# elizabethfong/SparkSmithWaterman

Hardware: AMD Instinct MI355X
Metric: GCUPS (higher is better)
Workload: dtype int32

## Files before the change

### sparksmithwaterman_amd/csrc/swmi_ctx.cpp

```cpp
#include <cstdarg>
#include <cstdio>
#include <cstdlib>

#include "swmi_host.h"
#include "swmi_launch.h"

static thread_local std::string g_err;

int swmi_host::fail(int code, const char *fmt, ...) {
    char buf[512];
    va_list ap;
    va_start(ap, fmt);
    vsnprintf(buf, sizeof buf, fmt, ap);
    va_end(ap);
    g_err = buf;
    return code;
}

int swmi_io_fail(int code, const std::string &msg) { return fail(code, "%s", msg.c_str()); }

static const uint8_t *code_table();

extern "C" int swmi_abi_version(void) { return SWMI_ABI_VERSION; }

// ... 131 lines not shown
        if (value != -1 && value != 1) return fail(SWMI_ERR_INVALID, "affine must be -1 (when gap_open != 0) or 1 (always)");
        ctx->affine = (int)value;
    } else if (!strcmp(name, "align_mode")) {
        if (value != SWMI_ALIGN_LOCAL && value != SWMI_ALIGN_FIT && value != SWMI_ALIGN_GLOBAL)
            return fail(SWMI_ERR_INVALID, "align_mode must be 0 (local), 1 (fit) or 2 (global), got %lld", (long long)value);
        ctx->modes.align_mode = (int)value;
    } else if (!strcmp(name, "long_reads")) {
        if (value != 0 && value != 1) return fail(SWMI_ERR_INVALID, "long_reads must be 0 or 1, got %lld", (long long)value);
        ctx->modes.long_reads = (int)value;
    } else if (!strcmp(name, "band")) {
        if (value < 0 || value > (int64_t)SWMI_AFF_BAND_MAX)
            return fail(SWMI_ERR_INVALID, "band must be 0 (none) or a half-width of 1 .. %u columns, got %lld", SWMI_AFF_BAND_MAX, (long long)value);
        ctx->modes.band = (int)value;
    } else if (!strcmp(name, "extend")) {
        if (value != 0 && value != 1) return fail(SWMI_ERR_INVALID, "extend must be 0 or 1, got %lld", (long long)value);
        ctx->modes.extend = (int)value;
    } else if (!strcmp(name, "xdrop")) {
        if (value < 0 || value > 0x7FFFFFFFll)
            return fail(SWMI_ERR_INVALID, "xdrop must be 0 (off) or a threshold of 1 .. 2^31 - 1, got %lld", (long long)value);
        ctx->modes.xdrop = (int)value;
    } else if (!strcmp(name, "band_adapt")) {
        if (value != 0 && value != 1) return fail(SWMI_ERR_INVALID, "band_adapt must be 0 or 1, got %lld", (long long)value);
        ctx->modes.band_adapt = (int)value;
    } else if (!strcmp(name, "arena_words_per_pair")) {
        if (value < 1) return fail(SWMI_ERR_INVALID, "arena_words_per_pair out of range");
        ctx->arena_words_per_pair = (uint64_t)value;
    } else {
        return fail(SWMI_ERR_INVALID, "unknown option '%s'", name);
    }
    return SWMI_OK;
}

extern "C" int swmi_set_score_matrix(swmi_ctx *ctx, const uint8_t *alphabet, uint32_t n, const int32_t *scores) {
    if (!ctx) return fail(SWMI_ERR_INVALID, "null context");
    if (n == 0) {
        std::lock_guard<std::mutex> g(ctx->mat_mu);
        ctx->matrix.reset();
        return SWMI_OK;
    }
    if (n > SWMI_MAT_MAX_SYMBOLS) return fail(SWMI_ERR_INVALID, "a score matrix has at most %u symbols, got %u", SWMI_MAT_MAX_SYMBOLS, n);
    if (!alphabet || !scores) return fail(SWMI_ERR_INVALID, "alphabet or scores is null");
    const uint8_t *T = code_table();
    uint32_t cls[256];
    for (uint32_t c = 0; c < 256; c++) cls[c] = n;
    for (uint32_t i = 0; i < n; i++) {
        const uint8_t c = T[alphabet[i]];
// ... 143 lines not shown
```

### sparksmithwaterman_amd/csrc/swmi_device.h

```cpp
#pragma once
#include <stdint.h>

#if defined(__HIPCC__)
#define SWMI_HD __host__ __device__
#else
#define SWMI_HD
#endif

#define SWMI_SEQ_PAD_WORDS 24u
#define SWMI_RMAX          4
#ifndef SWMI_CK_BLOCKS
#define SWMI_CK_BLOCKS     2u
#endif
#define SWMI_CODE_PAD      0x1FFu

#define SWMI_LDS_BYTES (160u * 1024u)
#define SWMI_EMIT_SCRATCH_WORDS 128u
#define SWMI_TB_BLOCKS 16u
#define SWMI_TB_REFWIN_WORDS 96u
#define SWMI_RES_CELL_CAP 128u

#define SWMI_DIR_D 0u
#define SWMI_DIR_I 1u
#define SWMI_DIR_A 2u

#define SWMI_F_DEGENERATE   0x1u
#define SWMI_F_CELL_OVF     0x2u
#define SWMI_F_ARENA_OVF    0x4u
#define SWMI_F_DONE         0x8u
#define SWMI_F_STRIPS_SHIFT 8u
#define SWMI_F_STRIPS_MASK  0xFFFFFF00u

struct SeqDesc {
    uint32_t len;
    uint32_t boff;
    uint32_t acgt;
    uint32_t pad;
};

struct PairDesc {
    uint32_t ref_id;
    uint32_t read_id;
// ... 244 lines not shown
```

### sparksmithwaterman_amd/csrc/swmi_diag.cpp

```cpp
#include <chrono>
#include <cstdio>
#include <cstdlib>
#include <unistd.h>

#include "swmi_host.h"

int swmi_host::dump_traceback_diagnostics(swmi_batch *b, const TraceArgs &ta, size_t np, size_t n_tf) {
    if (!ta.dbg) return SWMI_OK;
    std::vector<unsigned long long> d(np * 4);
    HIP_TRY(hipMemcpy(d.data(), ta.dbg, np * 32, hipMemcpyDeviceToHost));
    if (n_tf) {
        double t0 = 0, t1 = 0, t2 = 0, t3 = 0, t4 = 0, t5 = 0; unsigned long long mx = 0;
        for (size_t k = 0; k < np; k++) {
            t0 += d[4*k]; t1 += d[4*k+1] & 0xFFFFFFFFull; t2 += d[4*k+1] >> 32; t3 += d[4*k+2] >> 16; t4 += d[4*k+3] >> 32; t5 += d[4*k+3] & 0xFFFFFFFFull;
            mx = std::max(mx, d[4*k]);
        }
        fprintf(stderr, "[swmi tfused dbg] ticks per sweeper wavefront: lifetime mean=%.0f max=%llu = prologue %.0f + sweep %.0f + first block task %.0f (%.2f block tasks per wavefront) + waiting for tasks %.0f + rest (more tasks, walk items) %.0f\n",
                t0 / np, mx, t2 / np, t1 / np, t3 / np, t5 / np, t4 / np, (t0 - t1 - t2 - t3 - t4) / np);
        {
            std::vector<size_t> idx(np);
            for (size_t k = 0; k < np; k++) idx[k] = k;
            std::sort(idx.begin(), idx.end(), [&](size_t x, size_t y) { return d[4 * x] < d[4 * y]; });
            auto at = [&](double q) { return d[4 * idx[std::min<size_t>(np - 1, (size_t)(q * np))]]; };
            fprintf(stderr, "[swmi tfused dbg]   lifetime p10=%llu p50=%llu p90=%llu p99=%llu max=%llu\n", at(0.10), at(0.50), at(0.90), at(0.99), d[4 * idx[np - 1]]);
            for (size_t t = 0; t < std::min<size_t>(np, 6); t++) {
                const size_t k = idx[np - 1 - t];
                fprintf(stderr, "[swmi tfused dbg]   slow wavefront (pair %zu): lifetime %llu, sweep %llu, first block task %llu, block tasks taken %llu, waiting %llu, alignments of its pair %llu\n",
                        k, d[4 * k], d[4 * k + 1] & 0xFFFFFFFFull, d[4 * k + 2] >> 16, d[4 * k + 3] & 0xFFFFFFFFull, d[4 * k + 3] >> 32,
                        (unsigned long long)((const PairOut *)((const uint8_t *)b->h_result.p + result_out_off()))[k].n_cells);
            }
        }
    }
    double a0 = 0, a1 = 0, a2 = 0, a3 = 0; unsigned long long mx = 0;
    double a4 = 0;
    for (size_t k = 0; k < np; k++) { a0 += d[4*k]; a1 += d[4*k+1] & 0xFFFFFFFFull; a2 += d[4*k+2] & 0xFFFF; a4 += d[4*k+2] >> 16; a3 += d[4*k+3] & 0xFFFFFFFFull; mx = std::max(mx, d[4*k]); }
    fprintf(stderr, "[swmi tb dbg] wave ticks mean=%.0f max=%llu; walk ticks mean=%.0f; staging ticks mean=%.0f; steps mean=%.1f; iterations mean=%.2f\n",
            a0 / np, mx, a1 / np, a4 / np, a2 / np, a3 / np);
    const PairOut *po_dbg = (const PairOut *)((const uint8_t *)b->h_result.p + result_out_off());
    double cs[4] = {0, 0, 0, 0}, cw[4] = {0, 0, 0, 0}; unsigned long long cm[4] = {0, 0, 0, 0}; size_t cn[4] = {0, 0, 0, 0};
    for (size_t k = 0; k < np; k++) {
        const size_t c = std::min<uint64_t>(po_dbg[k].n_cells, 4) - (po_dbg[k].n_cells ? 1 : 0);
        cs[c] += d[4 * k]; cw[c] += d[4 * k + 1] & 0xFFFFFFFFull; cm[c] = std::max(cm[c], d[4 * k]); cn[c]++;
    }
    {
        std::vector<size_t> idx(np);
        for (size_t k = 0; k < np; k++) idx[k] = k;
        const size_t top = std::min<size_t>(np, 6);
        std::partial_sort(idx.begin(), idx.begin() + top, idx.end(), [&](size_t x, size_t y) { return d[4 * x] > d[4 * y]; });
        for (size_t t = 0; t < top; t++)
            fprintf(stderr, "[swmi tb dbg]   slow pair %zu: ticks=%llu walk=%llu staging=%llu in %llu stagings, steps=%llu iterations=%llu alignments=%llu\n", idx[t],
                    d[4 * idx[t]], d[4 * idx[t] + 1] & 0xFFFFFFFFull, d[4 * idx[t] + 2] >> 16, d[4 * idx[t] + 3] >> 32, d[4 * idx[t] + 2] & 0xFFFF,
                    d[4 * idx[t] + 3] & 0xFFFFFFFFull, (unsigned long long)po_dbg[idx[t]].n_cells);
        for (size_t t = 0; t < top; t++)
            fprintf(stderr, "[swmi tb dbg]     ... of the staging time of pair %zu, %llu ticks waiting for helpers\n", idx[t], d[4 * idx[t] + 1] >> 32);
    }
    for (int c = 0; c < 4; c++)
        if (cn[c]) fprintf(stderr, "[swmi tb dbg]   %d%s alignment(s): %zu pairs, wave ticks mean=%.0f max=%llu, walk(slot 0) mean=%.0f\n",
                           c + 1, c == 3 ? "+" : "", cn[c], cs[c] / cn[c], cm[c], cw[c] / cn[c]);
    return SWMI_OK;
}

int swmi_host::dump_fill_diagnostics(swmi_batch *b, const FillArgs &fa, size_t np) {
    if (!fa.dbg) return SWMI_OK;
    std::vector<unsigned long long> d(np * 2);
    HIP_TRY(hipMemcpy(d.data(), fa.dbg, np * 16, hipMemcpyDeviceToHost));
#ifdef SWMI_STRIP_DIAG
    for (size_t k = 0; k < np && k < 8; k++)
        fprintf(stderr, "[swmi strip dbg] pair %zu: strip 0 lifetime %llu ticks, %llu waiting before publications; strip 1 lifetime %llu, "
                "%llu polls, %llu ticks in polls, %llu waiting for seam groups\n", k, d[2 * k] >> 32, d[2 * k] & 0xFFFFFFFFull,
                d[2 * k + 1] >> 40, (d[2 * k + 1] >> 32) & 0xFF, (d[2 * k + 1] >> 16) & 0xFFFF, d[2 * k + 1] & 0xFFFF);
#endif
    unsigned long long ev = 0, cyc = 0, evmax = 0, cmax = 0, cmin = ~0ull;
    for (size_t k = 0; k < np; k++) {
        ev += d[2 * k]; cyc += d[2 * k + 1];
        evmax = std::max(evmax, d[2 * k]); cmax = std::max(cmax, d[2 * k + 1]); cmin = std::min(cmin, d[2 * k + 1]);
    }
    fprintf(stderr, "[swmi fill dbg] pairs=%zu slow-path entries mean=%.1f max=%llu; wave ticks mean=%.0f min=%llu max=%llu\n",
// ... 32 lines not shown
```

### sparksmithwaterman_amd/csrc/swmi_host.h

```cpp
#pragma once
#include <hip/hip_runtime.h>

#include <algorithm>
#include <atomic>
#include <condition_variable>
#include <cstdint>
#include <cstring>
#include <memory>
#include <mutex>
#include <string>
#include <thread>
#include <type_traits>
#include <unordered_map>
#include <vector>

#include "../../include/swmi.h"
#include "swmi_device.h"
#include "swmi_io_internal.h"

namespace swmi_host __attribute__((visibility("hidden"))) {
int fail(int code, const char *fmt, ...);
int check_offsets(const uint64_t *off, uint32_t n, const char *what);
int upload_device(swmi_ctx *ctx, swmi_batch *b, hipStream_t st, const uint8_t *ref_src, const uint8_t *read_src);
int settle_raw(swmi_batch *b);
// ... 47 lines not shown
        return SWMI_OK;
    }
    void release() { if (p) (void)hipHostFree(p); p = nullptr; dp = nullptr; cap = 0; }
    PinnedBuf() = default;
    PinnedBuf(const PinnedBuf &) = delete;
    PinnedBuf &operator=(const PinnedBuf &) = delete;
    ~PinnedBuf() { release(); }
};

struct ScoreMatrix {
    uint64_t gen = 0;
    uint32_t n = 0;
    int32_t max_entry = 0;
    std::vector<uint32_t> image;
};

struct __attribute__((visibility("hidden"))) RunModes {
    int align_mode = SWMI_ALIGN_LOCAL;
    int long_reads = 0;
    int band = 0;
    int extend = 0;
    int xdrop = 0;
    int band_adapt = 0;
    uint32_t kernel_mode() const { return extend && align_mode == SWMI_ALIGN_GLOBAL ? 3u : (uint32_t)align_mode; }
    bool operator==(const RunModes &o) const { return memcmp(this, &o, sizeof(RunModes)) == 0; }
};
static_assert(std::has_unique_object_representations_v<RunModes>, "RunModes is compared bytewise: no padding, no floating point");
static inline int64_t swmi_adapt_low(uint64_t m, uint64_t n, int64_t gap_open, int64_t gap) {
    const int64_t ns = (int64_t)((m + SWMI_AFF_MAX_READ - 1) / SWMI_AFF_MAX_READ);
    return (2 * ns + 1) * gap_open + (ns * (int64_t)SWMI_AFF_MAX_READ + (int64_t)n) * gap;
}
static inline bool swmi_adapt_bound_ok(uint64_t m, uint64_t n, int64_t gap_open, int64_t gap) {
    return swmi_adapt_low(m, n, gap_open, gap) >= -((int64_t)1 << 30);
}
struct __attribute__((visibility("hidden"))) RunOptions {
    RunModes modes;
    std::shared_ptr<const ScoreMatrix> mat;
};

struct swmi_ctx {
    int device = 0;
    hipStream_t stream = nullptr;
    std::mutex mu;
    uint32_t cell_cap = 64;
    uint64_t max_workspace_bytes = 32ull << 30;
    int profiling = 0;
// ... 193 lines not shown
```

### sparksmithwaterman_amd/csrc/swmi_run.cpp

```cpp
#include <chrono>
#include <cstdio>
#include <cstdlib>
#include <functional>
#include <numeric>

#include "swmi_host.h"
#include "swmi_launch.h"
#include "swmi_plan.h"

static int keep_chunk_records(RunState &rs, const AlnRec *tab, uint64_t n_rec, const uint32_t *arena, uint64_t arena_cap, size_t lo) {
    swmi_batch *b = rs.b;
    if (rs.defer_copy && b->raw_chunks.empty()) {
        b->raw_ext = arena; b->rtab_ext = tab; b->raw_ext_records = n_rec; b->raw_ext_cap = arena_cap;
        b->raw_chunks.push_back(swmi_batch::RawChunk{0, 0, 0, (size_t)n_rec, lo, {}});
        return SWMI_OK;
    }
    uint64_t used = 0;
    for (uint64_t k = 0; k < n_rec; k++) {
        const uint64_t end = (((uint64_t)tab[k].off_hi << 32) | tab[k].off_lo) + rec_words(tab[k].n_ops, b->rec_strings);
        used = std::max(used, end);
    }
    if (used > arena_cap) return fail(SWMI_ERR_HIP, "record payloads overrun the arena");
    b->raw_chunks.push_back(swmi_batch::RawChunk{b->raw.size(), (size_t)used, b->rtab.size(), (size_t)n_rec, lo, {}});
    b->raw.insert(b->raw.end(), arena, arena + used);
// ... 100 lines not shown
    return SWMI_OK;
}

static int build_trace_args(RunState &rs, Launch &L) {
    swmi_ctx *ctx = rs.ctx;
    swmi_batch *b = rs.b;
    const ChunkPlan &plan = b->plan;
    const FillArgs &fa = rs.fa;
    int rc;
    TraceArgs &ta = rs.ta;
    ta.seqw = fa.seqw; ta.refs = fa.refs; ta.reads = fa.reads; ta.pairs = fa.pairs;
    ta.dir = fa.dir; ta.out = fa.out; ta.cells = fa.cells;
    ta.cells_off = fa.cells_off; ta.cells_cap = fa.cells_cap;
    ta.hdr = (ArenaHdr *)L.res;
    ta.arena = (uint32_t *)(L.res + L.a_off);
    ta.arena_cap_words = L.arena_cap;
    ta.rec_tab = (AlnRec *)(L.res + L.t_off);
    ta.rec_tab_cap = (uint32_t)std::min<uint64_t>(L.tab_cap, 0xFFFFFFFFu);
    ta.n_pairs = fa.n_pairs; ta.cell_cap = fa.cell_cap;
    ta.match = fa.match; ta.mismatch = fa.mismatch; ta.gap = fa.gap; ta.strict = fa.strict;
    ta.lds_words = (plan.max_path + 3) / 4 + 1;
    ta.seam = fa.seam;
    ta.mode = b->eff_mode;
    ta.pad2 = 0;
    ta.lds_read_words = (plan.max_read + 3) / 4 + 1;
    ta.out_host = nullptr;
    ta.ovf_host = (uint32_t *)ctx->h_err.dp + 4;
    ((volatile uint32_t *)ctx->h_err.p)[4] = 0u; ((volatile uint32_t *)ctx->h_err.p)[5] = 0u;
    ta.win_off = nullptr; ta.q_count = nullptr; ta.q_items = nullptr; ta.q_cap = 0; ta.pad4 = 0;
    const bool strings = ctx->device_strings != 0 && b->d_raw.p != nullptr;
    ta.raw = strings ? b->d_raw.as<uint8_t>() : nullptr;
    ta.raw_off = strings ? b->d_raw_off.as<uint64_t>() : nullptr;
    ta.raw_reads_at = b->n_refs + 1u;
    b->rec_strings = strings;
    if (L.zc) {
        if ((rc = b->h_result.reserve(L.a_off + L.arena_cap * 4))) return rc;
        uint8_t *hd = (uint8_t *)b->h_result.dp;
        *(volatile uint32_t *)b->h_result.p = 0u;
        ((volatile uint32_t *)b->h_result.p)[1] = 0u;
        ta.ovf_host = (uint32_t *)hd;
        ta.out_host = (PairOut *)(hd + result_out_off());
        ta.arena = (uint32_t *)(hd + L.a_off);
        ta.rec_tab = (AlnRec *)(hd + L.t_off);
    }
    ta.dbg = nullptr;
    if (dbg_fill_on()) {
        if ((rc = b->d_dbg2.reserve(L.np * 32))) return rc;
        HIP_TRY(hipMemsetAsync(b->d_dbg2.p, 0, L.np * 32, ctx->stream));
        ta.dbg = b->d_dbg2.as<unsigned long long>();
    }
    L.whole_only = L.zc && plan.n_tf + plan.n_res == L.np;
    if (L.whole_only) {
        const uint32_t slots = 1024;
        if (!ctx->d_hdr_ring.p || ctx->hdr_next >= slots) {
            if ((rc = ctx->d_hdr_ring.reserve((size_t)slots * 64))) return rc;
            HIP_TRY(hipMemsetAsync(ctx->d_hdr_ring.p, 0, (size_t)slots * 64, ctx->stream));
            ctx->hdr_next = 0;
        }
        ta.hdr = (ArenaHdr *)(ctx->d_hdr_ring.as<uint8_t>() + (size_t)ctx->hdr_next++ * 64);
    }
    return SWMI_OK;
}

static ResidentArgs resident_args(const swmi_batch *b) {
    const ChunkPlan &plan = b->plan;
    ResidentArgs xa;
    xa.res_items = plan.n_res ? b->d_res_items.as<uint32_t>() : nullptr;
    xa.n_res = (uint32_t)plan.n_res; xa.res_lds_words = plan.res_lds_words; xa.res_cell_cap = SWMI_RES_CELL_CAP; xa.res_ops_words = plan.res_ops_words;
    return xa;
}

// ... 699 lines not shown
```

### sparksmithwaterman_amd/csrc/swmi_traceback.hip

```cpp
#include <hip/hip_runtime.h>
#include <hip/hip_ext.h>
#include <stdint.h>
#include <stdlib.h>
#include "swmi_device.h"
#include "swmi_emit.h"
#include "swmi_launch.h"
#include "swmi_walk.h"

template <int R>
__device__ __forceinline__ void coop_helper(const TraceArgs &A, const PairDesc pd, const uint32_t lane, const uint32_t wave,
                                            const uint32_t nw, const uint32_t ts, const uint32_t n_waves_all,
                                            uint32_t *__restrict__ tiles, volatile uint32_t *__restrict__ shared) {
    const SeqDesc rd = A.refs[pd.ref_id];
    const SeqDesc qd = A.reads[pd.read_id];
    const uint32_t n = rd.len, m = qd.len;
    const uint32_t *__restrict__ refw = A.seqw + rd.boff;
    const uint32_t *__restrict__ readw = A.seqw + qd.boff;
    const StripGeom G = strip_geom<R>(m, n, 1u);
    const bool acgt = rd.acgt && qd.acgt && SWMI_SCORES_FIT(A);
    const uint32_t team = (wave - nw) % nw, q = 1u + (wave - nw) / nw;
    uint32_t last = 0;
    for (;;) {
        uint32_t seq;
        while ((seq = __hip_atomic_load(const_cast<uint32_t *>(&shared[7u + 4u * team]), __ATOMIC_RELAXED, __HIP_MEMORY_SCOPE_WORKGROUP)) == last)
            __builtin_amdgcn_s_sleep(SWMI_HELPER_SLEEP);
        if (seq == 0xFFFFFFFFu) break;
        last = seq;
        __builtin_amdgcn_fence(__ATOMIC_ACQUIRE, "workgroup");
        const uint32_t flags = shared[4u + 4u * team], wlo = shared[5u + 4u * team], nq = shared[6u + 4u * team];
        const uint32_t s = flags >> 2;
        const uint32_t win = (flags & 2u) ? q - 1u : q;
        if (q < ts && win < nq) {
            uint32_t *__restrict__ base = ((flags & 1u) ? tiles + n_waves_all * (SWMI_CK_BLOCKS * SWMI_RMAX * WAVE) : tiles) +
                                          team * ts * (SWMI_CK_BLOCKS * SWMI_RMAX * WAVE);
            (void)replay_any<R, false, false>(A, pd, n, m, acgt, refw, readw, G, s, wlo + win * SWMI_CK_BLOCKS, lane,
                                       base + win * SWMI_CK_BLOCKS * R * WAVE, 0, 0u, nullptr, 0u);
            __builtin_amdgcn_fence(__ATOMIC_RELEASE, "workgroup");
            if (lane == 0) atomicAdd(const_cast<uint32_t *>(&shared[20u + team]), 1u);
        }
    }
}

template <int TMODE>
__device__ __forceinline__ void traceback_entry(const TraceArgs &A, uint32_t *lds_all) {
    const uint32_t wave = threadIdx.x >> 6;
    const uint32_t pair = blockIdx.x * FILL_WAVES + wave;
    if (pair >= A.n_pairs) return;
    const uint32_t lane = threadIdx.x & 63u;
    const uint32_t slot = blockIdx.y;
    uint32_t *tb_lds = lds_all + wave * (A.lds_words + A.lds_read_words + SWMI_TB_REFWIN_WORDS +
                                         (TMODE == 0 ? SWMI_TB_BLOCKS : SWMI_CK_BLOCKS) * SWMI_RMAX * WAVE);
    uint32_t *tile = tb_lds + A.lds_words + A.lds_read_words + SWMI_TB_REFWIN_WORDS;
    const PairDesc pd = A.pairs[pair];
    const PairOut po = A.out[pd.out_id];
    if (A.out_host && slot == 0 && lane == 0) A.out_host[pd.out_id] = po;
    if (po.flags & (SWMI_F_DEGENERATE | SWMI_F_CELL_OVF)) return;
    if (po.n_cells <= slot) return;
// ... 119 lines not shown
    return (pre && wave == 0) ? wlo0 : 0xFFFFFFFFu;
}

extern "C" __global__ void __launch_bounds__(WAVE * SWMI_TB_WAVES) __attribute__((amdgpu_waves_per_eu(4, 4)))
sw_traceback_winmax_kernel(const TraceArgs A) {
    extern __shared__ uint32_t wm_lds[];
    const uint32_t pair = blockIdx.x;
    if (pair >= A.n_pairs) return;
    const uint32_t wave = threadIdx.x >> 6, lane = threadIdx.x & 63u;
    const PairDesc pd = A.pairs[pair];
    PairOut po = A.out[pd.out_id];
    if (finish_pair(A, pd, po) && wave == 0 && lane == 0) A.out[pd.out_id] = po;
    if (po.flags & (SWMI_F_DEGENERATE | SWMI_F_DONE)) {
        if (A.out_host && wave == 0 && lane == 0) A.out_host[pd.out_id] = po;
        return;
    }
    const uint32_t n_waves = blockDim.x >> 6;
    const uint32_t per_walker = A.lds_words + A.lds_read_words + SWMI_TB_REFWIN_WORDS;
    constexpr uint32_t WIN_WORDS = SWMI_CK_BLOCKS * SWMI_RMAX * WAVE;
    uint32_t *shared = wm_lds;
    uint32_t *tiles = wm_lds + 32;
    const uint32_t R = swmi_rows_per_lane(A.reads[pd.read_id].len);
    const uint32_t ccap = A.cells_cap ? A.cells_cap[pd.out_id] : A.cell_cap;
    const uint32_t tile_sets = A.pad2 ? 2u : 1u;
    uint32_t *tiles2 = A.pad2 ? tiles + n_waves * WIN_WORDS : nullptr;
    uint32_t *walker_lds0 = tiles + tile_sets * n_waves * WIN_WORDS;
    if (!swmi_common_pair(A, A.refs[pd.ref_id], A.reads[pd.read_id])) {
        if (wave == 0) {
            uint32_t c;
            if (R == 1)      c = detect_cells<1>(A, pd, po, lane, tiles);
            else if (R == 2) c = detect_cells<2>(A, pd, po, lane, tiles);
            else if (R == 3) c = detect_cells<3>(A, pd, po, lane, tiles);
            else             c = detect_cells<4>(A, pd, po, lane, tiles);
            if (lane == 0) {
                po.n_cells = c;
                if (c > ccap) po.flags |= SWMI_F_CELL_OVF;
                A.out[pd.out_id] = po;
                if (A.out_host) A.out_host[pd.out_id] = po;
                shared[0] = c;
            }
            asm volatile("s_waitcnt vmcnt(0)" ::: "memory");
        }
        __syncthreads();
        const uint32_t c = shared[0];
        uint32_t nwr = c < SWMI_TB_SLOTS ? c : SWMI_TB_SLOTS;
        if (nwr > n_waves) nwr = n_waves;
        if (c > ccap || wave >= nwr) return;
        po.n_cells = c;
        uint32_t *lds = walker_lds0 + wave * per_walker;
// ... 9 lines not shown
    else if (R == 2) pre_wlo = winmax_detect<2>(A, pd, po, lane, wave, n_waves, ccap, tiles, walker_lds0, per_walker, shared);
    else if (R == 3) pre_wlo = winmax_detect<3>(A, pd, po, lane, wave, n_waves, ccap, tiles, walker_lds0, per_walker, shared);
    else             pre_wlo = winmax_detect<4>(A, pd, po, lane, wave, n_waves, ccap, tiles, walker_lds0, per_walker, shared);
    const uint32_t cnt = shared[0];
    if (shared[3] != 1u) pre_wlo = 0xFFFFFFFFu;
    if (cnt > ccap || cnt == 0u) return;
    po.n_cells = cnt;
    uint32_t nw = cnt < SWMI_TB_SLOTS ? cnt : SWMI_TB_SLOTS;
    if (nw > n_waves) nw = n_waves;
    const uint32_t ts = n_waves / nw;
    if (ts == 1u) {
        if (wave >= nw) return;
        uint32_t *lds = walker_lds0 + wave * per_walker;
        uint32_t *tile = tiles + wave * WIN_WORDS;
        if (R == 1)      traceback_pair<1, 1, false, false>(A, pd, po, lane, wave, nw, lds, tile, nullptr, 1u, pre_wlo, true);
        else if (R == 2) traceback_pair<2, 1, false, false>(A, pd, po, lane, wave, nw, lds, tile, nullptr, 1u, pre_wlo, true);
        else if (R == 3) traceback_pair<3, 1, false, false>(A, pd, po, lane, wave, nw, lds, tile, nullptr, 1u, pre_wlo, true);
        else             traceback_pair<4, 1, false, false>(A, pd, po, lane, wave, nw, lds, tile, nullptr, 1u, pre_wlo, true);
        return;
    }
    if (wave < nw) {
        uint32_t *lds = walker_lds0 + wave * per_walker;
        uint32_t *tile = tiles + wave * ts * WIN_WORDS;
        uint32_t *tile2 = tiles2 ? tiles2 + wave * ts * WIN_WORDS : nullptr;
        if (R == 1)      traceback_pair<1, 1, true, false>(A, pd, po, lane, wave, nw, lds, tile, shared, ts, pre_wlo, true, nullptr, tile2);
        else if (R == 2) traceback_pair<2, 1, true, false>(A, pd, po, lane, wave, nw, lds, tile, shared, ts, pre_wlo, true, nullptr, tile2);
        else if (R == 3) traceback_pair<3, 1, true, false>(A, pd, po, lane, wave, nw, lds, tile, shared, ts, pre_wlo, true, nullptr, tile2);
        else             traceback_pair<4, 1, true, false>(A, pd, po, lane, wave, nw, lds, tile, shared, ts, pre_wlo, true, nullptr, tile2);
    } else {
        if (R == 1)      coop_helper<1>(A, pd, lane, wave, nw, ts, n_waves, tiles, shared);
        else if (R == 2) coop_helper<2>(A, pd, lane, wave, nw, ts, n_waves, tiles, shared);
        else if (R == 3) coop_helper<3>(A, pd, lane, wave, nw, ts, n_waves, tiles, shared);
        else             coop_helper<4>(A, pd, lane, wave, nw, ts, n_waves, tiles, shared);
    }
}

extern "C" __global__ void __launch_bounds__(WAVE * FILL_WAVES)
sw_traceback_kernel(const TraceArgs A) {
    extern __shared__ uint32_t tb_lds[];
    traceback_entry<0>(A, tb_lds);
}

extern "C" __global__ void __launch_bounds__(WAVE * FILL_WAVES)
sw_traceback_replay_kernel(const TraceArgs A) {
    extern __shared__ uint32_t tb_lds[];
    traceback_entry<1>(A, tb_lds);
}
// ... 307 lines not shown

extern "C" hipError_t swmi_launch_resident(const TraceArgs *a, const ResidentArgs *x, hipStream_t st) {
    if (x->n_res == 0) return hipSuccess;
    static const bool attr = [] { swmi_allow_big_lds(sw_resident_pairs_kernel); return true; }();
    (void)attr;
    hipLaunchKernelGGL(sw_resident_pairs_kernel, dim3((x->n_res + FILL_WAVES - 1) / FILL_WAVES), dim3(WAVE * FILL_WAVES),
                       (size_t)FILL_WAVES * x->res_lds_words * sizeof(uint32_t), st, *a, *x);
    return hipGetLastError();
}

extern "C" hipError_t swmi_launch_traceback(const TraceArgs *a, hipStream_t st, hipEvent_t ev_start, hipEvent_t ev_stop) {
    if (a->n_pairs == 0) return hipSuccess;
    const size_t tile = (size_t)(a->mode == 0 ? SWMI_TB_BLOCKS : SWMI_CK_BLOCKS) * SWMI_RMAX * WAVE;
    const size_t per_wave = (size_t)a->lds_words + a->lds_read_words + SWMI_TB_REFWIN_WORDS + tile;
    const dim3 block(WAVE * FILL_WAVES);
    if (a->mode == 1) {
        static int forced = getenv("SWMI_TB_WAVES") ? atoi(getenv("SWMI_TB_WAVES")) : 0;
        static int big = getenv("SWMI_TB_BIG") ? atoi(getenv("SWMI_TB_BIG")) : 10000;
        const uint32_t n_waves = forced ? (uint32_t)forced : (a->n_pairs <= 512u ? SWMI_TB_WAVES : a->n_pairs <= (uint32_t)big ? 4u : 1u);
        const size_t n_walkers = n_waves < SWMI_TB_SLOTS ? n_waves : SWMI_TB_SLOTS;
        const size_t tiles = (size_t)n_waves * SWMI_CK_BLOCKS * SWMI_RMAX * WAVE;
        size_t words = 32 + tiles + n_walkers * ((size_t)a->lds_words + a->lds_read_words + SWMI_TB_REFWIN_WORDS);
        static const int spec_opt = getenv("SWMI_TB_SPEC") ? atoi(getenv("SWMI_TB_SPEC")) : 1;
        TraceArgs t = *a;
        t.pad2 = (spec_opt && (spec_opt == 2 || a->n_pairs <= 384u) && n_waves > 1u && (words + tiles) * sizeof(uint32_t) <= 160u * 1024u) ? 1u : 0u;
        if (t.pad2) words += tiles;
        if (ev_start && ev_stop)
            hipExtLaunchKernelGGL(sw_traceback_winmax_kernel, dim3(a->n_pairs), dim3(WAVE * n_waves), (uint32_t)(words * sizeof(uint32_t)), st, ev_start, ev_stop, 0u, t);
        else
            hipLaunchKernelGGL(sw_traceback_winmax_kernel, dim3(a->n_pairs), dim3(WAVE * n_waves), words * sizeof(uint32_t), st, t);
    } else {
        const dim3 grid((a->n_pairs + FILL_WAVES - 1) / FILL_WAVES, SWMI_TB_SLOTS);
        if (a->mode == 0) hipLaunchKernelGGL(sw_traceback_kernel, grid, block, per_wave * FILL_WAVES * sizeof(uint32_t), st, *a);
        else              hipLaunchKernelGGL(sw_traceback_replay_kernel, grid, block, per_wave * FILL_WAVES * sizeof(uint32_t), st, *a);
    }
    return hipGetLastError();
}
```

### sparksmithwaterman_amd/csrc/swmi_walk.h

```cpp
#pragma once
#include <hip/hip_runtime.h>
#include <stdint.h>
#include "swmi_device.h"
#include "swmi_emit.h"
#include "swmi_cells.h"

#ifndef SWMI_HELPER_SLEEP
#define SWMI_HELPER_SLEEP 8
#endif

#define SWMI_TB_SLOTS 4u
#if SWMI_CK_BLOCKS > 2
#define SWMI_TB_WAVES 4u
#else
#define SWMI_TB_WAVES 8u
#endif

template <int R, bool STRICT>
__device__ __forceinline__ void replay_window_fast(const TraceArgs &A, const PairDesc pd, const uint32_t n, const uint32_t m,
                                                   const uint32_t *__restrict__ refw, const uint32_t *__restrict__ readw,
                                                   const uint32_t wlo, const uint32_t lane, uint32_t *__restrict__ lds_tile) {
    const uint32_t gm = (uint32_t)(-(int64_t)A.gap);
    const int one = 1;
    int h[R], g[R], hp[R], q[R];
    uint32_t acc[R];
    const uint32_t *__restrict__ ck = A.dir + pd.dir_off + (uint64_t)(wlo / SWMI_CK_BLOCKS) * (R + 2) * WAVE + lane;
    build_profiles<R>(q, readw, lane * R, m, A.match, A.mismatch);
#pragma unroll
    for (int k = 0; k < R; ++k) {
        h[k] = (int)ld_l2(ck + k * WAVE);
        hp[k] = (uint32_t)h[k] > gm ? (int)((uint32_t)h[k] - gm) : 0;
        g[k] = 0;
        acc[k] = 0;
    }
// ... 181 lines not shown
    const uint32_t *__restrict__ readw = A.seqw + qd.boff;
    const StripGeom G = strip_geom<R>(m, n, A.mode);
    const uint32_t rps = G.rps;
    const uint32_t *__restrict__ dirp = A.dir + pd.dir_off;
    const uint32_t umat = (uint32_t)A.match, umis = (uint32_t)A.mismatch, ugap = (uint32_t)A.gap;
    const int dec0 = A.match > A.mismatch ? A.match : A.mismatch;
    const bool dec_fits = dec0 <= 0x7FFFFFFF / 23 && A.gap <= 0x7FFFFFFF / 23;
    const uint32_t udec = !dec_fits ? 0xFFFFFFFFu : dec0 > 0 ? (uint32_t)dec0 : 0u;
    const uint32_t ugdec = !dec_fits ? 0xFFFFFFFFu : A.gap > 0 ? (uint32_t)A.gap : 0u;
    (void)udec; (void)ugdec;
    const bool acgt = rd.acgt && qd.acgt && SWMI_SCORES_FIT(A);
    const uint8_t *__restrict__ raw_ref = A.raw ? A.raw + A.raw_off[pd.ref_id] : nullptr;
    const uint8_t *__restrict__ raw_read = A.raw ? A.raw + A.raw_off[A.raw_reads_at + pd.read_id] : nullptr;

    uint32_t *lds_ops = lds;
    uint32_t *lds_read = lds_ops + A.lds_words;
    uint32_t *lds_ref = lds_read + A.lds_read_words;
    uint8_t *ops_b = reinterpret_cast<uint8_t *>(lds_ops);
    const uint8_t *read_b = reinterpret_cast<const uint8_t *>(lds_read);
    const uint8_t *ref_b = reinterpret_cast<const uint8_t *>(lds_ref);
    uint32_t req_seq = 0, req_expected = 0;
    uint32_t *tile_cur = lds_tile, *tile_alt = lds_tile_alt;
    uint32_t spec_wlo = 0xFFFFFFFFu, spec_hi = 0u, spec_rv0 = 0u, spec_rv1 = 0u;
    auto team_wait = [&]() {
        while (__hip_atomic_load(const_cast<uint32_t *>(&shared[20u + slot]), __ATOMIC_RELAXED, __HIP_MEMORY_SCOPE_WORKGROUP) < req_expected)
            __builtin_amdgcn_s_sleep(1);
        __builtin_amdgcn_fence(__ATOMIC_ACQUIRE, "workgroup");
    };
    auto team_request = [&](uint32_t flags, uint32_t first_block, uint32_t nq, uint32_t delivered) {
        ++req_seq;
        req_expected += delivered;
        if (lane == 0) {
            shared[4u + 4u * slot] = flags; shared[5u + 4u * slot] = first_block; shared[6u + 4u * slot] = nq;
            __builtin_amdgcn_fence(__ATOMIC_RELEASE, "workgroup");
            __hip_atomic_store(const_cast<uint32_t *>(&shared[7u + 4u * slot]), req_seq, __ATOMIC_RELAXED, __HIP_MEMORY_SCOPE_WORKGROUP);
        }
    };

    const unsigned long long tk0 = TB_DBG ? __builtin_amdgcn_s_memtime() : 0ull;
    unsigned long long tk_walk = 0, tk_stage = 0, n_steps = 0, n_iters = 0;
    if (!read_staged)
        for (uint32_t w = lane; w < (m + 3u) / 4u; w += WAVE) lds_read[w] = readw[w];

    const uint64_t cbase = A.cells_off ? A.cells_off[pd.out_id] : (uint64_t)pd.out_id * A.cell_cap;
    const uint32_t ncell = one ? 1u : (uint32_t)po.n_cells;
    const uint2 *__restrict__ cells = A.cells + cbase;

    for (uint32_t base = 0; base < ncell; base += WAVE) {
        const uint32_t idx = base + lane;
        uint2 mine = make_uint2(0, 0);
        if (one) { mine.x = one->y; mine.y = one->z; }
        else if (idx < ncell) { mine.x = ld_l2(&cells[idx].x); mine.y = ld_l2(&cells[idx].y); }
        const uint64_t mykey = A.strict ? (((uint64_t)(mine.x + mine.y) << 32) | mine.y)
                                        : (((uint64_t)mine.x << 32) | mine.y);
        uint32_t rank = (one || ncell > WAVE) ? SWMI_RANK_BY_CELL : 0u;
        if (ncell > 1 && ncell <= WAVE) {
            for (uint32_t o = 0; o < ncell; ++o) {
                uint2 c; c.x = ld_l2(&cells[o].x); c.y = ld_l2(&cells[o].y);
                const uint64_t kk = A.strict ? (((uint64_t)(c.x + c.y) << 32) | c.y) : (((uint64_t)c.x << 32) | c.y);
                rank += (kk < mykey) ? 1u : 0u;
            }
        }
        const uint32_t nhere = ncell - base < WAVE ? ncell - base : WAVE;

        for (uint32_t a = slot; a < nhere; a += nslots) {
            const uint32_t ci = __builtin_amdgcn_readlane((int)mine.x, a);
            const uint32_t cj = __builtin_amdgcn_readlane((int)mine.y, a);
            const uint32_t crank = __builtin_amdgcn_readlane((int)rank, a);

            uint32_t i = ci, j = cj;
            uint32_t score = (uint32_t)po.score;
            uint32_t n_ops = 0;
            int begin = 0;
            while ((int)score > 0 && i != 0u && j != 0u) {
                const unsigned long long ts0 = TB_DBG ? __builtin_amdgcn_s_memtime() : 0ull;
                const uint32_t s = (i - 1u) / rps;
                int rho = (int)((i - 1u) - s * rps);
                const uint32_t t_cur = j - 1u + (uint32_t)rho / R;
                const uint32_t whi = t_cur >> 4;
                uint32_t wlo, nb;
                if (TMODE == 0) {
                    wlo = whi >= SWMI_TB_BLOCKS - 1u ? whi - (SWMI_TB_BLOCKS - 1u) : 0u;
                    nb = whi - wlo + 1u;
                } else if (COOP) {
                    const uint32_t wtop = whi - whi % SWMI_CK_BLOCKS;
                    wlo = wtop >= (ts - 1u) * SWMI_CK_BLOCKS ? wtop - (ts - 1u) * SWMI_CK_BLOCKS : 0u;
                    nb = wtop + SWMI_CK_BLOCKS - wlo;
                } else {
                    wlo = whi - whi % SWMI_CK_BLOCKS;
                    nb = SWMI_CK_BLOCKS;
                }
                bool use_spec = false;
                if (COOP && spec_wlo != 0xFFFFFFFFu) {
                    const uint32_t wtop = whi - whi % SWMI_CK_BLOCKS;
                    if (s == 0u && wtop + SWMI_CK_BLOCKS == spec_hi) { use_spec = true; wlo = spec_wlo; nb = spec_hi - spec_wlo; }
                }
                const bool prestaged = TMODE == 1 && pre_wlo == wlo && s == 0u && !use_spec;
                pre_wlo = 0xFFFFFFFFu;
                const int clo = (int)(16u * wlo) - 63;
                const uint32_t cw0 = clo > 0 ? (uint32_t)clo >> 2 : 0u;
                const uint32_t cw1 = (16u * (wlo + nb) - 1u) >> 2;
                WAVE_SYNC();
                if (use_spec) {
                    const unsigned long long tq0 = TB_DBG ? __builtin_amdgcn_s_memtime() : 0ull;
                    team_wait();
                    if (TB_DBG) tk_walk += (__builtin_amdgcn_s_memtime() - tq0) << 32;
                    uint32_t *t = tile_cur; tile_cur = tile_alt; tile_alt = t;
                    lds_ref[lane] = spec_rv0;
                    if (lane + WAVE < SWMI_TB_REFWIN_WORDS) lds_ref[lane + WAVE] = spec_rv1;
                    WAVE_SYNC();
                } else if (!prestaged) {
                    const uint32_t rx0 = cw0 + lane, rx1 = rx0 + WAVE, rlim = (n + 3u) / 4u;
                    const uint32_t rv0 = (rx0 <= cw1 && rx0 < rlim) ? refw[rx0] : 0u;
                    const uint32_t rv1 = (rx1 <= cw1 && rx1 < rlim) ? refw[rx1] : 0u;
                    if (TMODE == 0) {
                        const uint32_t *__restrict__ src = dirp + s * G.strip_words + (uint64_t)wlo * R * WAVE + lane;
                        for (uint32_t x = 0; x < nb * R; ++x) tile_cur[x * WAVE + lane] = src[(uint64_t)x * WAVE];
                    } else {
                        if (COOP) {
                            team_wait();
                            const uint32_t nq = nb / SWMI_CK_BLOCKS;
                            team_request((tile_cur == lds_tile ? 0u : 1u) | (s << 2), wlo, nq, nq - 1u);
                        }
                        (void)replay_any<R, false, FULL>(A, pd, n, m, acgt, refw, readw, G, s, wlo, lane, tile_cur, 0, 0u, nullptr, 0u);
                    }
                    lds_ref[lane] = rv0;
                    if (lane + WAVE < SWMI_TB_REFWIN_WORDS) lds_ref[lane + WAVE] = rv1;
                    if (COOP) {
                        const unsigned long long tq0 = TB_DBG ? __builtin_amdgcn_s_memtime() : 0ull;
                        team_wait();
                        if (TB_DBG) tk_walk += (__builtin_amdgcn_s_memtime() - tq0) << 32;
                    }
                    WAVE_SYNC();
                }
                spec_wlo = 0xFFFFFFFFu;
                if (COOP && tile_alt != nullptr && ts > 1u && wlo > 0u && s == 0u) {
                    const uint32_t have = wlo / SWMI_CK_BLOCKS, nq = have < ts - 1u ? have : ts - 1u;
                    spec_hi = wlo;
                    spec_wlo = wlo - nq * SWMI_CK_BLOCKS;
                    const int sclo = (int)(16u * spec_wlo) - 63;
                    const uint32_t scw0 = sclo > 0 ? (uint32_t)sclo >> 2 : 0u, scw1 = (16u * spec_hi - 1u) >> 2;
                    const uint32_t rx0 = scw0 + lane, rx1 = rx0 + WAVE, rlim = (n + 3u) / 4u;
                    spec_rv0 = (rx0 <= scw1 && rx0 < rlim) ? refw[rx0] : 0u;
                    spec_rv1 = (rx1 <= scw1 && rx1 < rlim) ? refw[rx1] : 0u;
                    team_request((tile_alt == lds_tile ? 0u : 1u) | 2u, spec_wlo, nq, nq);
                }
                const int tmin = (int)(16u * wlo);
                const unsigned long long tw0 = TB_DBG ? __builtin_amdgcn_s_memtime() : 0ull;
                if (TB_DBG) { tk_stage += tw0 - ts0; n_iters += 1ull << 32; }

#ifdef SWMI_WALK_CHASE
                for (;;) {
                    if (TB_DBG) ++n_iters;
                    const uint32_t na = lane >> 3, nb = lane & 7u;
                    const int rho_x = rho - (int)na;
                    const uint32_t rx = rho_x > 0 ? (uint32_t)rho_x : 0u;
                    const uint32_t lx = rx / R, kx = rx - lx * R;
                    const uint32_t jj = j - nb;
                    const int tx = (int)jj - 1 + (int)lx;
                    const bool valid = rho_x >= 0 && j > nb && tx >= tmin;
// ... 161 lines not shown
                uint32_t *dst = A.arena + off;
                if (lane == 0) swmi_write_rec(A, rslot, pd.out_id, crank, begin, ci, cj, n_ops, off);
                if (lane < opw) dst[lane] = packed0;
                for (uint32_t w = lane + WAVE; w < opw; w += WAVE) dst[w] = pack16(w);
                if (A.raw) {
                    const uint32_t w = 64u * (ctop - 1u) + lane;
                    if (w < sw) { dst[w] = wr0; dst[sw + w] = wq0; }
                    strs.store_from(dst, ctop - 1u);
                }
            } else if (lane == 0) {
                atomicOr(&A.out[pd.out_id].flags, SWMI_F_ARENA_OVF);
                if (A.ovf_host) *A.ovf_host = 1u;
            }
            WAVE_SYNC();
        }
    }
    if (COOP && lane == 0)
        __hip_atomic_store(const_cast<uint32_t *>(&shared[7u + 4u * slot]), 0xFFFFFFFFu, __ATOMIC_RELAXED, __HIP_MEMORY_SCOPE_WORKGROUP);
    if (TB_DBG && lane == 0 && slot == 0) {
        A.dbg[4 * pd.out_id] = __builtin_amdgcn_s_memtime() - tk0;
        A.dbg[4 * pd.out_id + 1] = tk_walk;
        A.dbg[4 * pd.out_id + 2] = n_steps | (tk_stage << 16);
        A.dbg[4 * pd.out_id + 3] = n_iters;
    }
}
```

Before: 2563.

## Add adaptive traceback look-ahead policy with partial second tile set

Adds a traceback look-ahead policy (automatic, off, rule-based, always) that decides per staging whether to speculatively request helper waves to replay the next window. The decision uses a score-based estimate of how far the walk will go. When no look-ahead is warranted on the last alignment, the walker releases its helpers and continues alone. The second LDS tile set can now be partially sized to fit a smaller budget, which lets occupancy stay higher. This aims to cut wasted speculative replays and waits on helpers, but it adds a heuristic that may mispredict and changes how LDS is sized.

```diff
diff --git a/sparksmithwaterman_amd/csrc/swmi_ctx.cpp b/sparksmithwaterman_amd/csrc/swmi_ctx.cpp
--- a/sparksmithwaterman_amd/csrc/swmi_ctx.cpp
+++ b/sparksmithwaterman_amd/csrc/swmi_ctx.cpp
@@ -177,6 +177,10 @@
     } else if (!strcmp(name, "band_adapt")) {
         if (value != 0 && value != 1) return fail(SWMI_ERR_INVALID, "band_adapt must be 0 or 1, got %lld", (long long)value);
         ctx->modes.band_adapt = (int)value;
+    } else if (!strcmp(name, "tb_lookahead")) {
+        if (value < -1 || value > 2)
+            return fail(SWMI_ERR_INVALID, "tb_lookahead must be -1 (automatic), 0 (off), 1 (the look-ahead rule) or 2 (at every staging), got %lld", (long long)value);
+        ctx->modes.tb_lookahead = (int)value;
     } else if (!strcmp(name, "arena_words_per_pair")) {
         if (value < 1) return fail(SWMI_ERR_INVALID, "arena_words_per_pair out of range");
         ctx->arena_words_per_pair = (uint64_t)value;
diff --git a/sparksmithwaterman_amd/csrc/swmi_device.h b/sparksmithwaterman_amd/csrc/swmi_device.h
--- a/sparksmithwaterman_amd/csrc/swmi_device.h
+++ b/sparksmithwaterman_amd/csrc/swmi_device.h
@@ -18,6 +18,9 @@
 #define SWMI_EMIT_SCRATCH_WORDS 128u
 #define SWMI_TB_BLOCKS 16u
 #define SWMI_TB_REFWIN_WORDS 96u
+#define SWMI_TB_LA_RULE    1u
+#define SWMI_TB_LA_ALWAYS  2u
+#define SWMI_TB_LA_PRIOR_DEN 3
 #define SWMI_RES_CELL_CAP 128u
 
 #define SWMI_DIR_D 0u
diff --git a/sparksmithwaterman_amd/csrc/swmi_diag.cpp b/sparksmithwaterman_amd/csrc/swmi_diag.cpp
--- a/sparksmithwaterman_amd/csrc/swmi_diag.cpp
+++ b/sparksmithwaterman_amd/csrc/swmi_diag.cpp
@@ -7,8 +7,8 @@
 
 int swmi_host::dump_traceback_diagnostics(swmi_batch *b, const TraceArgs &ta, size_t np, size_t n_tf) {
     if (!ta.dbg) return SWMI_OK;
-    std::vector<unsigned long long> d(np * 4);
-    HIP_TRY(hipMemcpy(d.data(), ta.dbg, np * 32, hipMemcpyDeviceToHost));
+    std::vector<unsigned long long> d(np * 6);
+    HIP_TRY(hipMemcpy(d.data(), ta.dbg, np * 48, hipMemcpyDeviceToHost));
     if (n_tf) {
         double t0 = 0, t1 = 0, t2 = 0, t3 = 0, t4 = 0, t5 = 0; unsigned long long mx = 0;
         for (size_t k = 0; k < np; k++) {
@@ -53,6 +53,17 @@
                     d[4 * idx[t] + 3] & 0xFFFFFFFFull, (unsigned long long)po_dbg[idx[t]].n_cells);
         for (size_t t = 0; t < top; t++)
             fprintf(stderr, "[swmi tb dbg]     ... of the staging time of pair %zu, %llu ticks waiting for helpers\n", idx[t], d[4 * idx[t] + 1] >> 32);
+    }
+    {
+        unsigned long long iss = 0, used = 0, wasted = 0, waits = 0;
+        double left = 0, life = 0; size_t n_left = 0;
+        for (size_t k = 0; k < np; k++) {
+            const unsigned long long c = d[4 * np + 2 * k], t = d[4 * np + 2 * k + 1];
+            iss += c & 0xFFFF; used += (c >> 16) & 0xFFFF; wasted += (c >> 32) & 0xFFFF; waits += c >> 48;
+            if (t) { left += (double)t; life += (double)d[4 * k]; n_left++; }
+        }
+        fprintf(stderr, "[swmi tb dbg] look-aheads issued=%llu used=%llu wasted=%llu, waits for the team=%llu; helpers left early in %zu pairs, at tick mean=%.0f of a walker lifetime of mean=%.0f\n",
+                iss, used, wasted, waits, n_left, n_left ? left / n_left : 0.0, n_left ? life / n_left : 0.0);
     }
     for (int c = 0; c < 4; c++)
         if (cn[c]) fprintf(stderr, "[swmi tb dbg]   %d%s alignment(s): %zu pairs, wave ticks mean=%.0f max=%llu, walk(slot 0) mean=%.0f\n",
diff --git a/sparksmithwaterman_amd/csrc/swmi_host.h b/sparksmithwaterman_amd/csrc/swmi_host.h
--- a/sparksmithwaterman_amd/csrc/swmi_host.h
+++ b/sparksmithwaterman_amd/csrc/swmi_host.h
@@ -93,6 +93,7 @@
     int extend = 0;
     int xdrop = 0;
     int band_adapt = 0;
+    int tb_lookahead = -1;
     uint32_t kernel_mode() const { return extend && align_mode == SWMI_ALIGN_GLOBAL ? 3u : (uint32_t)align_mode; }
     bool operator==(const RunModes &o) const { return memcmp(this, &o, sizeof(RunModes)) == 0; }
 };
diff --git a/sparksmithwaterman_amd/csrc/swmi_run.cpp b/sparksmithwaterman_amd/csrc/swmi_run.cpp
--- a/sparksmithwaterman_amd/csrc/swmi_run.cpp
+++ b/sparksmithwaterman_amd/csrc/swmi_run.cpp
@@ -146,7 +146,7 @@
     ta.lds_words = (plan.max_path + 3) / 4 + 1;
     ta.seam = fa.seam;
     ta.mode = b->eff_mode;
-    ta.pad2 = 0;
+    ta.pad2 = (uint32_t)(b->opt.modes.tb_lookahead + 1);
     ta.lds_read_words = (plan.max_read + 3) / 4 + 1;
     ta.out_host = nullptr;
     ta.ovf_host = (uint32_t *)ctx->h_err.dp + 4;
@@ -169,8 +169,8 @@
     }
     ta.dbg = nullptr;
     if (dbg_fill_on()) {
-        if ((rc = b->d_dbg2.reserve(L.np * 32))) return rc;
-        HIP_TRY(hipMemsetAsync(b->d_dbg2.p, 0, L.np * 32, ctx->stream));
+        if ((rc = b->d_dbg2.reserve(L.np * 48))) return rc;
+        HIP_TRY(hipMemsetAsync(b->d_dbg2.p, 0, L.np * 48, ctx->stream));
         ta.dbg = b->d_dbg2.as<unsigned long long>();
     }
     L.whole_only = L.zc && plan.n_tf + plan.n_res == L.np;
diff --git a/sparksmithwaterman_amd/csrc/swmi_traceback.hip b/sparksmithwaterman_amd/csrc/swmi_traceback.hip
--- a/sparksmithwaterman_amd/csrc/swmi_traceback.hip
+++ b/sparksmithwaterman_amd/csrc/swmi_traceback.hip
@@ -28,11 +28,11 @@
         last = seq;
         __builtin_amdgcn_fence(__ATOMIC_ACQUIRE, "workgroup");
         const uint32_t flags = shared[4u + 4u * team], wlo = shared[5u + 4u * team], nq = shared[6u + 4u * team];
+        const bool spec = (flags & 2u) != 0u;
         const uint32_t s = flags >> 2;
-        const uint32_t win = (flags & 2u) ? q - 1u : q;
-        if (q < ts && win < nq) {
-            uint32_t *__restrict__ base = ((flags & 1u) ? tiles + n_waves_all * (SWMI_CK_BLOCKS * SWMI_RMAX * WAVE) : tiles) +
-                                          team * ts * (SWMI_CK_BLOCKS * SWMI_RMAX * WAVE);
+        uint32_t *__restrict__ base = (flags & 1u) ? tiles + (n_waves_all + team * swmi_tb_set2_windows(A.pad2, nw, ts)) * (SWMI_CK_BLOCKS * SWMI_RMAX * WAVE)
+                                                   : tiles + team * ts * (SWMI_CK_BLOCKS * SWMI_RMAX * WAVE);
+        for (uint32_t win = spec ? q - 1u : q; q < ts && win < nq; win += spec ? ts - 1u : ts) {
             (void)replay_any<R, false, false>(A, pd, n, m, acgt, refw, readw, G, s, wlo + win * SWMI_CK_BLOCKS, lane,
                                        base + win * SWMI_CK_BLOCKS * R * WAVE, 0, 0u, nullptr, 0u);
             __builtin_amdgcn_fence(__ATOMIC_RELEASE, "workgroup");
@@ -198,9 +198,8 @@
     uint32_t *tiles = wm_lds + 32;
     const uint32_t R = swmi_rows_per_lane(A.reads[pd.read_id].len);
     const uint32_t ccap = A.cells_cap ? A.cells_cap[pd.out_id] : A.cell_cap;
-    const uint32_t tile_sets = A.pad2 ? 2u : 1u;
     uint32_t *tiles2 = A.pad2 ? tiles + n_waves * WIN_WORDS : nullptr;
-    uint32_t *walker_lds0 = tiles + tile_sets * n_waves * WIN_WORDS;
+    uint32_t *walker_lds0 = tiles + (n_waves + ((A.pad2 >> 8) & 0xFFu)) * WIN_WORDS;
     if (!swmi_common_pair(A, A.refs[pd.ref_id], A.reads[pd.read_id])) {
         if (wave == 0) {
             uint32_t c;
@@ -256,7 +255,7 @@
     if (wave < nw) {
         uint32_t *lds = walker_lds0 + wave * per_walker;
         uint32_t *tile = tiles + wave * ts * WIN_WORDS;
-        uint32_t *tile2 = tiles2 ? tiles2 + wave * ts * WIN_WORDS : nullptr;
+        uint32_t *tile2 = tiles2 ? tiles2 + wave * swmi_tb_set2_windows(A.pad2, nw, ts) * WIN_WORDS : nullptr;
         if (R == 1)      traceback_pair<1, 1, true, false>(A, pd, po, lane, wave, nw, lds, tile, shared, ts, pre_wlo, true, nullptr, tile2);
         else if (R == 2) traceback_pair<2, 1, true, false>(A, pd, po, lane, wave, nw, lds, tile, shared, ts, pre_wlo, true, nullptr, tile2);
         else if (R == 3) traceback_pair<3, 1, true, false>(A, pd, po, lane, wave, nw, lds, tile, shared, ts, pre_wlo, true, nullptr, tile2);
@@ -610,9 +609,21 @@
         const size_t tiles = (size_t)n_waves * SWMI_CK_BLOCKS * SWMI_RMAX * WAVE;
         size_t words = 32 + tiles + n_walkers * ((size_t)a->lds_words + a->lds_read_words + SWMI_TB_REFWIN_WORDS);
         static const int spec_opt = getenv("SWMI_TB_SPEC") ? atoi(getenv("SWMI_TB_SPEC")) : 1;
+        uint32_t policy = a->pad2 ? a->pad2 - 1u : a->n_pairs <= 384u ? SWMI_TB_LA_ALWAYS : n_waves > 4u ? SWMI_TB_LA_RULE : 0u;
+        if (spec_opt != 1) policy = spec_opt == 2 ? SWMI_TB_LA_ALWAYS : 0u;
+        if (n_waves == 1u) policy = 0u;
+        const size_t win_words = (size_t)SWMI_CK_BLOCKS * SWMI_RMAX * WAVE;
+        uint32_t set2 = 0;
+        if (policy == SWMI_TB_LA_ALWAYS || (policy == SWMI_TB_LA_RULE && n_waves > 4u)) {
+            if ((words + tiles) * sizeof(uint32_t) <= 160u * 1024u) set2 = n_waves;
+        } else if (policy == SWMI_TB_LA_RULE) {
+            const size_t budget = 15u * 1280u / sizeof(uint32_t);
+            while (set2 < n_waves && words + (set2 + 1u) * win_words <= budget) ++set2;
+        }
+        if (set2 == 0u) policy = 0u;
         TraceArgs t = *a;
-        t.pad2 = (spec_opt && (spec_opt == 2 || a->n_pairs <= 384u) && n_waves > 1u && (words + tiles) * sizeof(uint32_t) <= 160u * 1024u) ? 1u : 0u;
-        if (t.pad2) words += tiles;
+        t.pad2 = policy ? policy | (set2 << 8) : 0u;
+        words += set2 * win_words;
         if (ev_start && ev_stop)
             hipExtLaunchKernelGGL(sw_traceback_winmax_kernel, dim3(a->n_pairs), dim3(WAVE * n_waves), (uint32_t)(words * sizeof(uint32_t)), st, ev_start, ev_stop, 0u, t);
         else
diff --git a/sparksmithwaterman_amd/csrc/swmi_walk.h b/sparksmithwaterman_amd/csrc/swmi_walk.h
--- a/sparksmithwaterman_amd/csrc/swmi_walk.h
+++ b/sparksmithwaterman_amd/csrc/swmi_walk.h
@@ -10,6 +10,10 @@
 #endif
 
 #define SWMI_TB_SLOTS 4u
+__device__ __forceinline__ uint32_t swmi_tb_set2_windows(uint32_t pad2, uint32_t nw, uint32_t ts) {
+    const uint32_t per_team = ((pad2 >> 8) & 0xFFu) / nw;
+    return per_team < ts ? per_team : ts;
+}
 #if SWMI_CK_BLOCKS > 2
 #define SWMI_TB_WAVES 4u
 #else
@@ -237,6 +241,9 @@
     uint32_t req_seq = 0, req_expected = 0;
     uint32_t *tile_cur = lds_tile, *tile_alt = lds_tile_alt;
     uint32_t spec_wlo = 0xFFFFFFFFu, spec_hi = 0u, spec_rv0 = 0u, spec_rv1 = 0u;
+    const uint32_t la_policy = COOP ? (A.pad2 & 0xFFu) : 0u;
+    const uint32_t la_cap = swmi_tb_set2_windows(A.pad2, nslots, ts);
+    bool alone = false;
     auto team_wait = [&]() {
         while (__hip_atomic_load(const_cast<uint32_t *>(&shared[20u + slot]), __ATOMIC_RELAXED, __HIP_MEMORY_SCOPE_WORKGROUP) < req_expected)
             __builtin_amdgcn_s_sleep(1);
@@ -254,6 +261,7 @@
 
     const unsigned long long tk0 = TB_DBG ? __builtin_amdgcn_s_memtime() : 0ull;
     unsigned long long tk_walk = 0, tk_stage = 0, n_steps = 0, n_iters = 0;
+    unsigned long long la_cnt = 0, la_left = 0;
     if (!read_staged)
         for (uint32_t w = lane; w < (m + 3u) / 4u; w += WAVE) lds_read[w] = readw[w];
 
@@ -287,6 +295,9 @@
             uint32_t score = (uint32_t)po.score;
             uint32_t n_ops = 0;
             int begin = 0;
+            const uint32_t t_first = cj - 1u + ((ci - 1u) % rps) / R;
+            const bool last_aln = a + nslots >= nhere && base + WAVE >= ncell;
+            (void)t_first; (void)last_aln;
             while ((int)score > 0 && i != 0u && j != 0u) {
                 const unsigned long long ts0 = TB_DBG ? __builtin_amdgcn_s_memtime() : 0ull;
                 const uint32_t s = (i - 1u) / rps;
@@ -297,7 +308,7 @@
                 if (TMODE == 0) {
                     wlo = whi >= SWMI_TB_BLOCKS - 1u ? whi - (SWMI_TB_BLOCKS - 1u) : 0u;
                     nb = whi - wlo + 1u;
-                } else if (COOP) {
+                } else if (COOP && !alone) {
                     const uint32_t wtop = whi - whi % SWMI_CK_BLOCKS;
                     wlo = wtop >= (ts - 1u) * SWMI_CK_BLOCKS ? wtop - (ts - 1u) * SWMI_CK_BLOCKS : 0u;
                     nb = wtop + SWMI_CK_BLOCKS - wlo;
@@ -319,7 +330,7 @@
                 if (use_spec) {
                     const unsigned long long tq0 = TB_DBG ? __builtin_amdgcn_s_memtime() : 0ull;
                     team_wait();
-                    if (TB_DBG) tk_walk += (__builtin_amdgcn_s_memtime() - tq0) << 32;
+                    if (TB_DBG) { tk_walk += (__builtin_amdgcn_s_memtime() - tq0) << 32; la_cnt += 1ull << 16; }
                     uint32_t *t = tile_cur; tile_cur = tile_alt; tile_alt = t;
                     lds_ref[lane] = spec_rv0;
                     if (lane + WAVE < SWMI_TB_REFWIN_WORDS) lds_ref[lane + WAVE] = spec_rv1;
@@ -332,8 +343,11 @@
                         const uint32_t *__restrict__ src = dirp + s * G.strip_words + (uint64_t)wlo * R * WAVE + lane;
                         for (uint32_t x = 0; x < nb * R; ++x) tile_cur[x * WAVE + lane] = src[(uint64_t)x * WAVE];
                     } else {
-                        if (COOP) {
+                        if (TB_DBG && spec_wlo != 0xFFFFFFFFu) la_cnt += 1ull << 32;
+                        if (COOP && !alone) {
+                            if (TB_DBG) la_cnt += 1ull << 48;
                             team_wait();
+                            if (tile_cur != lds_tile) { tile_alt = tile_cur; tile_cur = lds_tile; }
                             const uint32_t nq = nb / SWMI_CK_BLOCKS;
                             team_request((tile_cur == lds_tile ? 0u : 1u) | (s << 2), wlo, nq, nq - 1u);
                         }
@@ -341,7 +355,7 @@
                     }
                     lds_ref[lane] = rv0;
                     if (lane + WAVE < SWMI_TB_REFWIN_WORDS) lds_ref[lane + WAVE] = rv1;
-                    if (COOP) {
+                    if (COOP && !alone) {
                         const unsigned long long tq0 = TB_DBG ? __builtin_amdgcn_s_memtime() : 0ull;
                         team_wait();
                         if (TB_DBG) tk_walk += (__builtin_amdgcn_s_memtime() - tq0) << 32;
@@ -349,8 +363,26 @@
                     WAVE_SYNC();
                 }
                 spec_wlo = 0xFFFFFFFFu;
-                if (COOP && tile_alt != nullptr && ts > 1u && wlo > 0u && s == 0u) {
-                    const uint32_t have = wlo / SWMI_CK_BLOCKS, nq = have < ts - 1u ? have : ts - 1u;
+                bool ahead = COOP && !alone && tile_alt != nullptr && ts > 1u && wlo > 0u && s == 0u;
+                uint32_t la_nq = ts - 1u;
+                if (COOP && !alone && la_policy == SWMI_TB_LA_RULE && tile_alt != nullptr && ts > 1u) {
+                    la_nq = la_cap;
+                    if (ahead && la_nq != 0u) {
+                        const uint32_t left = t_cur + 1u - 16u * wlo, gone = t_first - t_cur, shed = (uint32_t)po.score - score;
+                        ahead = gone >= 16u * SWMI_CK_BLOCKS ? score * gone > shed * left
+                                                             : score * (uint32_t)((R + 1) * SWMI_TB_LA_PRIOR_DEN) > umat * (uint32_t)R * left;
+                    }
+                    ahead = ahead && la_nq != 0u;
+                    if (!ahead && last_aln) {
+                        alone = true;
+                        if (TB_DBG) la_left = __builtin_amdgcn_s_memtime() - tk0;
+                        if (lane == 0)
+                            __hip_atomic_store(const_cast<uint32_t *>(&shared[7u + 4u * slot]), 0xFFFFFFFFu, __ATOMIC_RELAXED, __HIP_MEMORY_SCOPE_WORKGROUP);
+                    }
+                }
+                if (ahead) {
+                    if (TB_DBG) la_cnt += 1ull;
+                    const uint32_t have = wlo / SWMI_CK_BLOCKS, nq = have < la_nq ? have : la_nq;
                     spec_hi = wlo;
                     spec_wlo = wlo - nq * SWMI_CK_BLOCKS;
                     const int sclo = (int)(16u * spec_wlo) - 63;
@@ -558,5 +590,9 @@
         A.dbg[4 * pd.out_id + 1] = tk_walk;
         A.dbg[4 * pd.out_id + 2] = n_steps | (tk_stage << 16);
         A.dbg[4 * pd.out_id + 3] = n_iters;
-    }
-}
+        if (COOP) {
+            A.dbg[4 * A.n_pairs + 2 * pd.out_id] = la_cnt + (spec_wlo != 0xFFFFFFFFu ? 1ull << 32 : 0ull);
+            A.dbg[4 * A.n_pairs + 2 * pd.out_id + 1] = la_left;
+        }
+    }
+}
```

After: 2554. No clear change (-0.4%).
